# gardner-lab/syllable-detector-swift

Hardware: AMD Instinct MI355X
Metric: audio frames/sec (256-pt STFT + 2-layer MLP), whole job (higher is better)
Workload: dtype f32 (I/O and accumulate; products as f16 hi/lo split x3 on MFMA)

## Files before the change

syllable_detector_swift_amd/csrc/kernels_fused_s.hip:

```cpp

#include "fused_common.hpp"

namespace sd {

namespace {

using namespace fused_dev;

constexpr int kTile = kFusedSTileFrames;

typedef __attribute__((address_space(3))) void lds_void;

__device__ __forceinline__ float rem_lo(float a, unsigned h)
{
    float r;
    asm("v_fma_mix_f32 %0, %1, 1.0, -%2 op_sel_hi:[0,0,1]" : "=v"(r) : "v"(a), "v"(h));
    return r;
}
__device__ __forceinline__ float rem_hi(float a, unsigned h)
{
    float r;
    asm("v_fma_mix_f32 %0, %1, 1.0, -%2 op_sel:[0,0,1] op_sel_hi:[0,0,1]" : "=v"(r) : "v"(a), "v"(h));
    return r;
}
__device__ __forceinline__ unsigned cvt_pk(float a, float b)
{
    unsigned r;
    asm("v_cvt_pk_f16_f32 %0, %1, %2" : "=v"(r) : "v"(a), "v"(b));
    return r;
}
__device__ __forceinline__ floatx4 s16x4(const int16_t *p)
{
    const uint2 v = *reinterpret_cast<const uint2 *>(p);
    constexpr float k = 1.0f / 32768.0f;
    return floatx4{(float)(int16_t)(v.x & 0xffffu) * k, (float)((int)v.x >> 16) * k, (float)(int16_t)(v.y & 0xffffu) * k,
                   (float)((int)v.y >> 16) * k};
}
__device__ __forceinline__ float s16x1(const int16_t *p) { return (float)p[0] * (1.0f / 32768.0f); }

__device__ __forceinline__ void split2(float a, float b, unsigned &hi, unsigned &lo)
{
    hi = cvt_pk(a, b);
    lo = cvt_pk(rem_lo(a, hi), rem_hi(b, hi));
}

template <int K2, bool GEN, int HQ, int NW, int PADP = 0, bool F2 = false, int NT = 1, bool SPECT = false, bool MN = false, bool S16 = false>
__global__ void __launch_bounds__(64 * NW, 1)
fused_s_kernel(const FusedDesc d, const float *__restrict__ samples, int64_t stride, int64_t s_eff, int64_t E,
               float *__restrict__ outputs, uint8_t *__restrict__ flags, const FusedNet *__restrict__ nets, const int *__restrict__ net_of,
               const int *__restrict__ row_of)
{
    static_assert(!(MN && SPECT), "the spectrogram instantiation runs no network");
    static_assert(!S16 || (K2 == 4 && F2 && PADP == 0 && NT == 1 && HQ == 1 && NW == 8 && !SPECT), "16-bit PCM: the twice-folded form on the plain ring");
    extern __shared__ __attribute__((aligned(16))) unsigned char smem[];
    const int tid = threadIdx.x;
    const int lane = tid & 63;
    const int wave = __builtin_amdgcn_readfirstlane(tid >> 6);
    const int n = lane & 15, g = lane >> 4;
    constexpr int kWaves = NW;
    const int c = blockIdx.y;
    const int T = d.T, H = d.H, hop = d.hop;
    constexpr int W = 64 * K2;
    const int n_out = GEN ? d.n_out : 1;
    const int64_t e_b = ((int64_t)blockIdx.x * kWaves + wave) * d.s_seg_evals;
    if (e_b >= E) return;
    const int64_t e_e = (e_b + d.s_seg_evals < E) ? e_b + d.s_seg_evals : E;
    const int seg_len = (int)(e_e - e_b);
    const int tiles = (seg_len + (T - 1) + kTile - 1) / kTile;
    const unsigned e_b32 = (unsigned)e_b;
    const FusedNet *nt = MN ? nets + __builtin_amdgcn_readfirstlane(net_of[c]) : nullptr;
#define SD_NET(f) (MN ? nt->f : d.f)

    const int fr = d.s_perm ? (n < 4 ? 2 * n : (n >= 12 ? 2 * (n - 8) : 2 * (n - 4) + 1)) : n;

    unsigned char *wbase = smem + (size_t)wave * d.s_lds_wave;
    const int RC = PADP == 1 ? d.s_cs8_rc : d.s_ring_chunks, R = RC * (S16 ? 512 : 256);
    constexpr bool CS8 = PADP == 1;
    static_assert(!CS8 || (F2 && HQ == 1 && NT == 1), "staggered chunks: the twice-folded form at hop 128");
    constexpr int kSub = PADP > 1 ? 256 / PADP : 1;
    constexpr int kChunkB = CS8 ? 1280 : 1024 + (PADP > 1 ? 16 * kSub : 0);
    auto sk = [](int i) { return PADP > 1 ? 4 * (i / (PADP > 1 ? PADP : 1)) : 0; };
    float *ring = reinterpret_cast<float *>(wbase);
    const int16_t *ring16 = reinterpret_cast<const int16_t *>(wbase);
    const int PS = d.s_pstride, TP = d.s_tp;
    float *rows = reinterpret_cast<float *>(wbase + (size_t)(RC + (CS8 ? 0 : 1)) * kChunkB);
    float *zquad = rows + (T - 1 + kTile) * PS;
    constexpr bool kTbl = HQ == 2 && NW == 8;
    float *gtab = zquad + 8 * HQ + 32 * g;
    {
        const int nz = ((T - 1 + kTile) * PS + 8 * HQ + 128) / 4;
        for (int i = lane; i < nz; i += 64) reinterpret_cast<floatx4 *>(rows)[i] = floatx4{0.f, 0.f, 0.f, 0.f};
    }

    constexpr int KB = F2 ? 1 : K2;
    half8 as_[KB][2][2], ad_[KB][2][2];
    if (!F2) {
#pragma unroll
        for (int ks = 0; ks < KB; ks++)
#pragma unroll
            for (int m = 0; m < 2; m++)
#pragma unroll
                for (int p = 0; p < 2; p++) {
                    as_[ks][m][p] = as_half8(reinterpret_cast<const uint32x4 *>(d.sfrag)[(((ks * 2 + 0) * 2 + m) * 2 + p) * 64 + lane]);
                    ad_[ks][m][p] = as_half8(reinterpret_cast<const uint32x4 *>(d.sfrag)[(((ks * 2 + 1) * 2 + m) * 2 + p) * 64 + lane]);
                }
    }
    half8 b2[F2 ? 2 : 1][F2 ? 4 * NT : 1][2];
    float w1c[F2 ? 16 : 1], w2c[F2 ? 16 : 1], ce[4 * NT], w192 = 0.0f;
#pragma unroll
    for (int i = 0; i < 4 * NT; i++) ce[i] = 0.0f;
    if (F2) {
#pragma unroll
        for (int ks = 0; ks < 2; ks++)
#pragma unroll
            for (int gm = 0; gm < 4; gm++)
#pragma unroll
                for (int tau = 0; tau < NT; tau++)
#pragma unroll
                    for (int p = 0; p < 2; p++)
                        b2[ks][gm + 4 * tau][p] = as_half8(reinterpret_cast<const uint32x4 *>(d.sfrag2)[(((ks * 4 + gm) * NT + tau) * 2 + p) * 64 + lane]);
#pragma unroll
        for (int i = 0; i < 16; i++) {
            w1c[i] = d.swin2[(g * 16 + i) * 2];
            w2c[i] = d.swin2[(g * 16 + i) * 2 + 1];
        }
#pragma unroll
        for (int i = 0; i < 4 * NT; i++) ce[i] = d.s2c[lane * 16 + i];
        w192 = d.s2c[lane * 16 + 8];
    }
    half8 aft[3][HQ][NT][2];
#pragma unroll
    for (int m = 0; m < 3; m++)
#pragma unroll
        for (int q = 0; q < HQ; q++)
#pragma unroll
            for (int tau = 0; tau < NT; tau++)
#pragma unroll
                for (int p = 0; p < 2; p++)
                    aft[m][q][tau][p] = as_half8(reinterpret_cast<const uint32x4 *>(F2 ? (HQ == 1 ? SD_NET(afrag_t2) : SD_NET(afrag_w2)) : (HQ == 1 ? SD_NET(afrag_t) : SD_NET(afrag_w)))[(((m * HQ + q) * NT + tau) * 2 + p) * 64 + lane]);
    float cre[8];
#pragma unroll
    for (int i = 0; i < 8; i++) cre[i] = F2 ? 0.0f : d.slone[lane * 8 + i];
    if (kTbl && n == 0) {
#pragma unroll
        for (int i = 0; i < 8; i++) gtab[i] = cre[i];
    }

    const int rc = MN ? bank_row(row_of, c) : c;
    const float *row = S16 ? reinterpret_cast<const float *>(reinterpret_cast<const int16_t *>(samples) + (int64_t)rc * stride)
                           : samples + (int64_t)rc * stride;
    const __amdgpu_buffer_rsrc_t in_rs = __builtin_amdgcn_make_buffer_rsrc(const_cast<float *>(row), 0, (int)(s_eff * (S16 ? 2 : 4)), 0x00020000);
    const __amdgpu_buffer_rsrc_t out_rs = __builtin_amdgcn_make_buffer_rsrc(
        outputs ? outputs + (int64_t)rc * E * n_out : nullptr, 0, outputs ? (int)(E * n_out * 4) : 0, 0x00020000);
    const __amdgpu_buffer_rsrc_t flg_rs = __builtin_amdgcn_make_buffer_rsrc(flags ? flags + (int64_t)rc * E : nullptr, 0, flags ? (int)E : 0, 0x00020000);
    const __amdgpu_buffer_rsrc_t spc_rs = __builtin_amdgcn_make_buffer_rsrc(
        SPECT ? d.spect_out + (int64_t)c * E * d.F : nullptr, 0, SPECT ? (int)(E * d.F * 4) : 0, 0x00020000);

    const unsigned org = (unsigned)((e_b * hop + d.gap) * (S16 ? 2 : 4));
    int cn = 0, slot = 0;
    auto issue_upto = [&](int last) {
        while (cn <= last) {
            const unsigned voff = org + (unsigned)cn * 1024u + (unsigned)lane * 16u;
            if (CS8) {
                const int pad = ((cn & 6) << 1) | (cn & 1);
                __builtin_amdgcn_raw_ptr_buffer_load_lds(in_rs, (lds_void *)(wbase + slot * kChunkB + 16 * pad), 16, voff, 0, 0, 2 );
            } else if (PADP == 0) {
                __builtin_amdgcn_raw_ptr_buffer_load_lds(in_rs, (lds_void *)(wbase + slot * 1024), 16, voff, 0, 0, 2 );
                if (slot == 0) __builtin_amdgcn_raw_ptr_buffer_load_lds(in_rs, (lds_void *)(wbase + RC * 1024), 16, voff, 0, 0, 2);
            } else {
#pragma unroll
                for (int k = 0; k < kSub; k++)
                    if (lane / (64 / kSub) == k) {
                        __builtin_amdgcn_raw_ptr_buffer_load_lds(in_rs, (lds_void *)(wbase + slot * kChunkB + 16 * k), 16, voff, 0, 0, 2);
                        if (slot == 0) __builtin_amdgcn_raw_ptr_buffer_load_lds(in_rs, (lds_void *)(wbase + RC * kChunkB + 16 * k), 16, voff, 0, 0, 2);
                    }
            }
            cn++;
            slot = slot + 1 == RC ? 0 : slot + 1;
        }
    };
    const int span = (kTile - 1) * hop + W;
    constexpr int kChunkLog = S16 ? 9 : 8;
    auto need = [&](int t) { return (kTile * hop * t + span - 1) >> kChunkLog; };
    auto allowed = [&](int t) { return RC - 1 + ((kTile * hop * t) >> kChunkLog); };

    unsigned fo = (unsigned)(hop * fr);
    unsigned sb1 = (unsigned)((fr >> 1) * kChunkB), sb2 = (unsigned)(((fr >> 1) + (fr & 1)) * kChunkB);
    const int jq1 = (fr >> 1) & 7, jq2 = ((fr >> 1) + (fr & 1)) & 7;
    const unsigned cb1 = (unsigned)(16 * (((jq1 & 6) << 1) | (jq1 & 1)) + ((fr & 1) ? 512 : 0));
    const unsigned cb2 = (unsigned)(16 * (((jq2 & 6) << 1) | (jq2 & 1)) + ((fr & 1) ? 0 : 512));
    float *prow = rows + (T - 1 + fr) * PS;
    const float *erow = rows + n * PS;
    const float *pv_p[3], *sv_p[3];
#pragma unroll
    for (int tt = 0; tt < 3; tt++) {
        const int t = g + 4 * tt;
        pv_p[tt] = t < T ? erow + t * PS + 4 * HQ * t : zquad;
        sv_p[tt] = t < T ? erow + t * PS + 4 * HQ * TP : zquad;
    }
    float *pt_p[3];
#pragma unroll
    for (int m = 0; m < 3; m++) pt_p[m] = 4 * m + g < TP ? prow + 4 * HQ * (4 * m + g) : zquad + 4 * HQ;

    const float c_b1 = GEN ? (g < n_out ? SD_NET(b1)[g] : 0.0f) : SD_NET(b1)[0];
    float lean_oa = 0.0f, lean_og = 1.0f, lean_ob = 0.0f;
    if (d.n_out_fns == 1) {
        const int o = (GEN && g < n_out) ? g : 0;
        lean_oa = SD_NET(out_params)[0]; lean_og = SD_NET(out_params)[1 + o]; lean_ob = SD_NET(out_params)[1 + n_out + o];
    }
    float b0g[HQ], w1g[HQ], w1o[4][HQ], rvg[HQ];
#pragma unroll
    for (int q = 0; q < HQ; q++) {
        const int u = 4 * q + g;
        rvg[q] = (GEN && u < H) ? SD_NET(rvec)[u] : 0.0f;
        b0g[q] = u < H ? SD_NET(bias0)[u] : 0.0f;
        w1g[q] = u < H ? SD_NET(w1)[u] : 0.0f;
#pragma unroll
        for (int o = 0; o < 4; o++) w1o[o][q] = (GEN && u < H && o < n_out) ? SD_NET(w1)[o * H + u] : 0.0f;
    }
    if (kTbl && n == 0) {
#pragma unroll
        for (int q = 0; q < HQ; q++) {
            gtab[8 + q] = b0g[q];
            gtab[8 + HQ + q] = w1g[q];
            gtab[8 + 6 * HQ + q] = rvg[q];
#pragma unroll
            for (int o = 0; o < 4; o++) gtab[8 + 2 * HQ + o * HQ + q] = w1o[o][q];
        }
    }
    const bool multi = GEN && n_out > 1;
    const double thr_g = SD_NET(thresholds)[(GEN && g < n_out) ? g : 0];
    if (kTbl && n == 0) {
        gtab[22] = c_b1; gtab[23] = lean_oa; gtab[24] = lean_og; gtab[25] = lean_ob;
        *reinterpret_cast<double *>(gtab + 26) = thr_g;
    }
    const bool counts = !GEN || n_out == 1 ? true : (g < n_out && (g == 0 || d.rule == 1));
    const int tf0 = GEN ? d.tf0 : 0, tf1 = GEN ? d.tf1 : 2, norm = GEN ? d.norm : 1;
    const int scaling = GEN ? d.scaling : 0;
    const float klog = scaling == 1 ? 0.6931471805599453f : 6.020599913279624f;
    bool binv[8 * NT];
#pragma unroll
    for (int i = 0; i < 8 * NT; i++) {
        const int tau = i >> 3, ii = i & 7;
        binv[i] = (F2 ? 32 * tau + (ii < 4 ? 8 * g + d.s2_pe + 2 * ii : 8 * g + d.s2_po + 2 * (ii - 4)) : (ii < 4 ? 4 * g + ii : 16 + 4 * g + (ii - 4))) < d.F;
    }
    const float kmag = pow2f(-13 - d.col_shift);
    const bool guard_on = d.fix.counters != nullptr;
    const float guard_k = norm == 1 ? SD_NET(guard_r) : (norm == 0 ? SD_NET(guard_rel_r) : SD_NET(guard_range_r));
    const float mn_wu = MN ? nt->w_unscale : 0.0f, mn_loud = MN ? nt->guard_loud : 0.0f;
    const int mn_se_abs = MN ? nt->guard_se_abs_r : 0;
#undef SD_NET

    issue_upto(need(0) < allowed(0) ? need(0) : allowed(0));
    int se_ref = 0;

#ifdef SYLDET_S_STAMPS
    unsigned long long st_vm = 0, st_lg = 0;
    const unsigned long long st_begin = __builtin_amdgcn_s_memtime();
#define SD_STAMP(var, stmt) { asm volatile("s_waitcnt lgkmcnt(0)" ::: "memory"); const unsigned long long t0_ = __builtin_amdgcn_s_memtime(); stmt; \
                              const unsigned long long t1_ = __builtin_amdgcn_s_memtime(); var += t1_ - t0_; }
#else
#define SD_STAMP(var, stmt) { stmt; }
#endif
#ifndef SYLDET_S_NO_PREWAIT
    __builtin_amdgcn_s_waitcnt(0x0F70);
#endif
#if defined(SYLDET_S_SETPRIO_SECOND)
    if (wave >= kWaves / 2) __builtin_amdgcn_s_setprio(1);
#elif defined(SYLDET_S_SETPRIO_FIRST)
    if (wave < kWaves / 2) __builtin_amdgcn_s_setprio(1);
#endif
    for (int t = 0; t < tiles; t++) {
        SD_STAMP(st_vm, if (t == 0) asm volatile("s_waitcnt vmcnt(0)" ::: "memory"); else if (SPECT) asm volatile("s_waitcnt vmcnt(5)" ::: "memory");
                        else asm volatile("s_waitcnt vmcnt(2)" ::: "memory"));
        const float *f1 = reinterpret_cast<const float *>(wbase + sb1 + cb1);
        const float *f2 = reinterpret_cast<const float *>(wbase + sb2 + cb2);
        const float *fp = CS8 ? f1 : ring + fo + sk((int)fo);

        floatx4 P1[2][2], P3[2][2], P2[2][2], P4[2][2];
        float P2w[2], P4w[2], x64 = 0.0f, x192 = 0.0f;
        if (F2) {
#pragma unroll
            for (int ks = 0; ks < 2; ks++) {
                if (CS8) {
                    const float *a1 = f1 + 32 * ks + 8 * g, *a2 = f2 + 32 * ks + 8 * g;
                    const float *b1 = f1 + 120 - 32 * ks - 8 * g, *b3 = f2 + 120 - 32 * ks - 8 * g;
                    P1[ks][0] = *reinterpret_cast<const floatx4 *>(a1);
                    P1[ks][1] = *reinterpret_cast<const floatx4 *>(a1 + 4);
                    P3[ks][0] = *reinterpret_cast<const floatx4 *>(a2);
                    P3[ks][1] = *reinterpret_cast<const floatx4 *>(a2 + 4);
                    P2[ks][0] = *reinterpret_cast<const floatx4 *>(b1);
                    P2[ks][1] = *reinterpret_cast<const floatx4 *>(b1 + 4);
                    P2w[ks] = (ks == 0) ? (g == 0 ? f2 : b1 + 8)[0] : b1[8];
                    P4[ks][0] = *reinterpret_cast<const floatx4 *>(b3);
                    P4[ks][1] = *reinterpret_cast<const floatx4 *>(b3 + 4);
                    P4w[ks] = b3[8];
                    continue;
                }
                if (S16) {
                    const int16_t *a = ring16 + fo + 32 * ks + 8 * g, *b = ring16 + fo + 120 - 32 * ks - 8 * g;
                    P1[ks][0] = s16x4(a);
                    P1[ks][1] = s16x4(a + 4);
                    P3[ks][0] = s16x4(a + 128);
                    P3[ks][1] = s16x4(a + 132);
                    P2[ks][0] = s16x4(b);
                    P2[ks][1] = s16x4(b + 4);
                    P2w[ks] = s16x1(b + 8);
                    P4[ks][0] = s16x4(b + 128);
                    P4[ks][1] = s16x4(b + 132);
                    P4w[ks] = s16x1(b + 136);
                    continue;
                }
                const float *a = fp + 32 * ks + 8 * g, *b = fp + 120 - 32 * ks - 8 * g;
                P1[ks][0] = *reinterpret_cast<const floatx4 *>(a);
                P1[ks][1] = *reinterpret_cast<const floatx4 *>(a + 4);
                P3[ks][0] = *reinterpret_cast<const floatx4 *>(a + 128 + sk(128));
                P3[ks][1] = *reinterpret_cast<const floatx4 *>(a + 132 + sk(128));
                P2[ks][0] = *reinterpret_cast<const floatx4 *>(b + sk(64));
                P2[ks][1] = *reinterpret_cast<const floatx4 *>(b + 4 + sk(64));
                P2w[ks] = (PADP && ks == 0) ? b[8 + (g == 0 ? sk(128) : sk(64))] : b[8 + sk(64)];
                P4[ks][0] = *reinterpret_cast<const floatx4 *>(b + 128 + sk(192));
                P4[ks][1] = *reinterpret_cast<const floatx4 *>(b + 132 + sk(192));
                P4w[ks] = b[136 + sk(192)];
            }
            x64 = S16 ? s16x1(ring16 + fo + 64) : (CS8 ? f1[64] : fp[64 + sk(64)]);
            x192 = S16 ? s16x1(ring16 + fo + 192) : (CS8 ? f2[64] : fp[192 + sk(192)]);
            SD_STAMP(st_lg, asm volatile("s_waitcnt lgkmcnt(0)" ::: "memory"));
            if (t + 1 < tiles) issue_upto(need(t + 1));
        }
        float amax;
#ifdef SYLDET_S_NOMAX
        amax = 1.0f;
#else
        {
            float m0 = 0.0f, m1 = 0.0f;
            if (F2) {
#pragma unroll
                for (int ks = 0; ks < 2; ks++)
#pragma unroll
                    for (int h = 0; h < 2; h++) {
                        m0 = absmax3(m0, P1[ks][h][0], P1[ks][h][1]);
                        m1 = absmax3(m1, P1[ks][h][2], P1[ks][h][3]);
                        m0 = absmax3(m0, P3[ks][h][0], P3[ks][h][1]);
                        m1 = absmax3(m1, P3[ks][h][2], P3[ks][h][3]);
                        m0 = absmax3(m0, P2[ks][h][0], P2[ks][h][1]);
                        m1 = absmax3(m1, P2[ks][h][2], P2[ks][h][3]);
                        m0 = absmax3(m0, P4[ks][h][0], P4[ks][h][1]);
                        m1 = absmax3(m1, P4[ks][h][2], P4[ks][h][3]);
                    }
                m0 = absmax3(m0, P2w[0], P2w[1]);
                m1 = absmax3(m1, g == 0 ? 0.0f : P4w[0], P4w[1]);
                m0 = absmax3(m0, x64, x192);
            } else {
                const floatx4 *q0 = reinterpret_cast<const floatx4 *>(fp + (W / 4) * g + sk((W / 4) * g));
#pragma unroll
                for (int q = 0; q < W / 16; q++) {
                    const floatx4 v = q0[q];
                    m0 = absmax3(m0, v[0], v[1]);
                    m1 = absmax3(m1, v[2], v[3]);
                }
            }
            amax = fmaxf(m0, m1);
            auto r = __builtin_amdgcn_permlane16_swap(__float_as_uint(amax), __float_as_uint(amax), false, false);
            amax = fmaxf(__uint_as_float(r[0]), __uint_as_float(r[1]));
            r = __builtin_amdgcn_permlane32_swap(__float_as_uint(amax), __float_as_uint(amax), false, false);
            amax = fmaxf(__uint_as_float(r[0]), __uint_as_float(r[1]));
        }
#endif
        const int ex = (int)((__float_as_uint(amax) >> 23) & 0xffu);
        int se = (F2 ? 139 : 140) - ex;
        const int fst = amax > 0.0f ? ((ex == 255 || se < -100) ? 2 : 0) : 1;
        se = amax > 0.0f ? (se < -100 ? -100 : (se > 113 ? 113 : se)) : 0;
        const float sx = pow2f(se);
        if (t == 0) {
            const float tm = wave_max_nonneg(amax);
            const int exr = (int)((__float_as_uint(tm) >> 23) & 0xffu);
            int r0 = (F2 ? 139 : 140) - exr;
            r0 = tm > 0.0f ? (r0 < -100 ? -100 : (r0 > 113 ? 113 : r0)) : 0;
            se_ref = __builtin_amdgcn_readfirstlane(r0);
        }

        if (!F2 && t + 1 < tiles) issue_upto(need(t + 1) < allowed(t) ? need(t + 1) : allowed(t));

        const float xl = S16 ? 0.0f : fp[0] * sx;
        floatx4 acc[4 * NT];
#pragma unroll
        for (int i = 0; i < 4 * NT; i++) acc[i] = floatx4{0.f, 0.f, 0.f, 0.f};
        float a64 = 0.0f;
        const float *xpb = fp + W / 2 + 8 * g, *xmb = fp + W / 2 - 8 * g;
        const float *xmz = xmb + ((PADP && g == 0) ? 4 : 0);
#ifndef SYLDET_S_NODFT
        if (F2) {
            a64 = w192 * fmaf(x192, sx, x64 * sx);
            const float b64 = w192 * fmaf(x192, sx, -(x64 * sx));
#pragma unroll
            for (int ks = 0; ks < 2; ks++) {
                const float xa[8] = {P3[ks][0][0], P3[ks][0][1], P3[ks][0][2], P3[ks][0][3], P3[ks][1][0], P3[ks][1][1], P3[ks][1][2], P3[ks][1][3]};
                const float xd[8] = {P1[ks][0][0], P1[ks][0][1], P1[ks][0][2], P1[ks][0][3], P1[ks][1][0], P1[ks][1][1], P1[ks][1][2], P1[ks][1][3]};
                const float xb[8] = {P2w[ks], P2[ks][1][3], P2[ks][1][2], P2[ks][1][1], P2[ks][1][0], P2[ks][0][3], P2[ks][0][2], P2[ks][0][1]};
                const float xc[8] = {P4w[ks], P4[ks][1][3], P4[ks][1][2], P4[ks][1][1], P4[ks][1][0], P4[ks][0][3], P4[ks][0][2], P4[ks][0][1]};
                float ap[8], am[8], bm[8], bp[8];
#pragma unroll
                for (int i = 0; i < 8; i++) {
                    const float t1 = xb[i] * sx, t2 = xd[i] * sx;
                    float s1 = fmaf(xa[i], sx, t1), d1 = fmaf(xa[i], sx, -t1);
                    float s2 = fmaf(xc[i], sx, t2), d2 = fmaf(xc[i], sx, -t2);
                    if (ks == 0 && i == 0) {
                        s1 = g == 0 ? xa[0] * sx : s1;
                        s2 = g == 0 ? t2 : s2;
                    }
                    const float w1 = w1c[ks * 8 + i], w2 = w2c[ks * 8 + i];
                    const float p = w2 * s2, q = w2 * d2;
                    ap[i] = fmaf(w1, s1, p);
                    am[i] = fmaf(w1, s1, -p);
                    bm[i] = fmaf(w1, d1, -q);
                    bp[i] = fmaf(w1, d1, q);
                }
                if (ks == 0) {
                    bm[0] = g == 0 ? 0.0f : bm[0];
                    bp[0] = g == 0 ? b64 : bp[0];
                }
                uint32x4 vh[4], vl[4];
#pragma unroll
                for (int j = 0; j < 4; j++) {
                    unsigned h, l;
                    split2(ap[2 * j], ap[2 * j + 1], h, l);
                    vh[0][j] = h; vl[0][j] = l;
                    split2(am[2 * j], am[2 * j + 1], h, l);
                    vh[1][j] = h; vl[1][j] = l;
                    split2(bm[2 * j], bm[2 * j + 1], h, l);
                    vh[2][j] = h; vl[2][j] = l;
                    split2(bp[2 * j], bp[2 * j + 1], h, l);
                    vh[3][j] = h; vl[3][j] = l;
                }
#pragma unroll
                for (int gm = 0; gm < 4 * NT; gm++) acc[gm] = mfma(b2[ks][gm][0], as_half8(vh[gm & 3]), acc[gm]);
#pragma unroll
                for (int gm = 0; gm < 4 * NT; gm++) acc[gm] = mfma(b2[ks][gm][0], as_half8(vl[gm & 3]), acc[gm]);
#pragma unroll
                for (int gm = 0; gm < 4 * NT; gm++) acc[gm] = mfma(b2[ks][gm][1], as_half8(vh[gm & 3]), acc[gm]);
            }
        } else {
#pragma unroll
        for (int ks = 0; ks < KB; ks++) {
            const int skp = sk(W / 2 + 32 * ks), skm = sk(W / 2 - 32 * ks - 32), skw = sk(W / 2 - 32 * ks);
            const floatx4 p0 = *reinterpret_cast<const floatx4 *>(xpb + 32 * ks + skp), p1 = *reinterpret_cast<const floatx4 *>(xpb + 32 * ks + 4 + skp);
            const floatx4 q1 = *reinterpret_cast<const floatx4 *>(xmb - 32 * ks - 8 + skm), q2 = *reinterpret_cast<const floatx4 *>(xmb - 32 * ks - 4 + skm);
            const float q0 = (skw != skm ? xmz : xmb)[-32 * ks + skm];
            const float xp[8] = {p0[0], p0[1], p0[2], p0[3], p1[0], p1[1], p1[2], p1[3]};
            const float xm[8] = {q0, q2[3], q2[2], q2[1], q2[0], q1[3], q1[2], q1[1]};
            float s[8], dd[8];
#pragma unroll
            for (int i = 0; i < 8; i++) {
                const float tm = xm[i] * sx;
                s[i] = fmaf(xp[i], sx, tm);
                dd[i] = fmaf(xp[i], sx, -tm);
            }
            if (ks == 0) dd[0] = g == 0 ? xl : dd[0];
            uint32x4 sh, sl, dh, dl;
#pragma unroll
            for (int j = 0; j < 4; j++) {
                unsigned h, l;
                split2(s[2 * j], s[2 * j + 1], h, l);
                sh[j] = h; sl[j] = l;
                split2(dd[2 * j], dd[2 * j + 1], h, l);
                dh[j] = h; dl[j] = l;
            }
            const half8 bsh = as_half8(sh), bsl = as_half8(sl), bdh = as_half8(dh), bdl = as_half8(dl);
#pragma unroll
            for (int m = 0; m < 2; m++) acc[m] = mfma(as_[ks][m][0], bsh, acc[m]);
#pragma unroll
            for (int m = 0; m < 2; m++) acc[2 + m] = mfma(ad_[ks][m][0], bdh, acc[2 + m]);
#pragma unroll
            for (int m = 0; m < 2; m++) acc[m] = mfma(as_[ks][m][0], bsl, acc[m]);
#pragma unroll
            for (int m = 0; m < 2; m++) acc[2 + m] = mfma(ad_[ks][m][0], bdl, acc[2 + m]);
#pragma unroll
            for (int m = 0; m < 2; m++) acc[m] = mfma(as_[ks][m][1], bsh, acc[m]);
#pragma unroll
            for (int m = 0; m < 2; m++) acc[2 + m] = mfma(ad_[ks][m][1], bdh, acc[2 + m]);
        }
        }
#else
        acc[0][0] = xpb[0]; acc[1][1] = xmb[0];
#endif
        if (!F2) {
            SD_STAMP(st_lg, asm volatile("s_waitcnt lgkmcnt(0)" ::: "memory"));
            if (t + 1 < tiles) issue_upto(need(t + 1));
        }

        float cval[8 * NT], mss = 0.0f;
        float cre_l[8];
        if (kTbl) {
            const float *tp = gtab;
            asm volatile("" : "+v"(tp));
            const floatx4 c0 = *reinterpret_cast<const floatx4 *>(tp), c1 = *reinterpret_cast<const floatx4 *>(tp + 4);
#pragma unroll
            for (int i = 0; i < 4; i++) { cre_l[i] = c0[i]; cre_l[4 + i] = c1[i]; }
        } else {
#pragma unroll
            for (int i = 0; i < 8; i++) cre_l[i] = cre[i];
        }
#pragma unroll
        for (int i = 0; i < 8 * NT; i++) {
            const int tau = i >> 3, ii = i & 7;
            const float re = F2 ? (ii < 4 ? fmaf(ce[4 * tau + ii], a64, acc[4 * tau][ii]) : acc[4 * tau + 1][ii & 3]) : fmaf(cre_l[ii], xl, acc[ii >> 2][ii & 3]);
            const float im = F2 ? (ii < 4 ? acc[4 * tau + 2][ii] : acc[4 * tau + 3][ii & 3]) : acc[2 + (ii >> 2)][ii & 3];
            cval[i] = __builtin_amdgcn_sqrtf(fmaf(re, re, im * im)) * kmag;
        }
        if constexpr (SPECT) {
            static_assert(NT == 1 && F2, "the spectrogram instantiation is the twice-folded one");
            const int er = kTile * t + fr;
            const bool vld = er < seg_len;
            const int ush = d.col_shift - se;
            const float up = pow2f(ush < -126 ? -126 : (ush > 126 ? 126 : ush));
            const unsigned rowo = (e_b32 + (unsigned)er) * (unsigned)d.F;
            const bool odd_first = d.s2_pe != 0;
            float v8[8];
#pragma unroll
            for (int i = 0; i < 4; i++) {
                const float me = cval[i] * up, mo = cval[4 + i] * up;
                const float a = odd_first ? mo : me, b = odd_first ? me : mo;
                v8[2 * i] = d.spect_power ? a * a : a;
                v8[2 * i + 1] = d.spect_power ? b * b : b;
            }
            const int fq = d.F >> 2, rem = d.F & 3;
#pragma unroll
            for (int q = 0; q < 2; q++) {
                const int Q = 2 * g + q;
                const uint32x4 w = {__float_as_uint(v8[4 * q]), __float_as_uint(v8[4 * q + 1]), __float_as_uint(v8[4 * q + 2]), __float_as_uint(v8[4 * q + 3])};
                __builtin_amdgcn_raw_buffer_store_b128(w, spc_rs, (vld && Q < fq) ? (rowo + 4u * (unsigned)Q) * 4u : 0xFFFFFFFFu, 0, 0);
            }
            {
                const bool mine = vld && (fq >> 1) == g;
#pragma unroll
                for (int j = 0; j < 3; j++) {
                    const float pv = (fq & 1) ? v8[4 + j] : v8[j];
                    __builtin_amdgcn_raw_buffer_store_b32(__float_as_uint(pv), spc_rs, (mine && j < rem) ? (rowo + 4u * (unsigned)fq + (unsigned)j) * 4u : 0xFFFFFFFFu, 0, 0);
                }
            }
            if (guard_on && __builtin_amdgcn_ballot_w64(vld && fst == 2) != 0ull) {
                const int lo = kTile * t, hi = lo + kTile < seg_len ? lo + kTile : seg_len;
                if (lane == 0 && hi > lo) {
                    const unsigned sl = atomicAdd(d.fix.counters, 1u);
                    if (sl < d.fix.capacity) d.fix.items[sl] = FixItem{c, e_b32 + (unsigned)lo, hi - lo, 1};
                    else d.fix.counters[3] = 1u;
                }
            }
            fo += (unsigned)(kTile * hop);
            fo = fo >= (unsigned)R ? fo - (unsigned)R : fo;
            if (CS8) {
                sb1 += 8u * kChunkB; sb1 = sb1 >= (unsigned)(RC * kChunkB) ? sb1 - (unsigned)(RC * kChunkB) : sb1;
                sb2 += 8u * kChunkB; sb2 = sb2 >= (unsigned)(RC * kChunkB) ? sb2 - (unsigned)(RC * kChunkB) : sb2;
            }
            continue;
        }
        if (GEN && scaling != 0) {
            const float off = (float)(d.col_shift - se) * klog;
#pragma unroll
            for (int i = 0; i < 8 * NT; i++) cval[i] = binv[i] ? fmaf(__builtin_amdgcn_logf(cval[i]), klog, off) : 0.0f;
        }
#pragma unroll
        for (int i = 0; i < 8 * NT; i++) mss = fmaf(cval[i], cval[i], mss);
        mss = xor32_sum(xor16_sum(mss));
        int dsc = (GEN && scaling != 0) ? 0 : se_ref - se;
        const bool far = dsc > 45 || dsc < -45 || fst == 2;
        dsc = dsc < -45 ? -45 : (dsc > 45 ? 45 : dsc);
        unsigned tb = ((__float_as_uint(mss) + 0x800000u) >> 1) & 0x7f800000u;
        tb = (unsigned)min(max((int)tb, 16 << 23), 80 << 23);
        const float fs_up = __uint_as_float((203u << 23) - tb);
        const float fs_ring = __uint_as_float(tb + ((unsigned)(dsc + 51) << 23));
        uint32x4 bh[NT], bl[NT];
#pragma unroll
        for (int j = 0; j < 4 * NT; j++) {
            unsigned h, l;
            split2(cval[2 * j] * fs_up, cval[2 * j + 1] * fs_up, h, l);
            bh[j >> 2][j & 3] = h; bl[j >> 2][j & 3] = l;
        }
        floatx4 pt[3][HQ];
#pragma unroll
        for (int m = 0; m < 3; m++)
#pragma unroll
            for (int q = 0; q < HQ; q++) {
                pt[m][q] = floatx4{0.f, 0.f, 0.f, 0.f};
#pragma unroll
                for (int tau = 0; tau < NT; tau++) {
                    pt[m][q] = mfma(aft[m][q][tau][0], as_half8(bh[tau]), pt[m][q]);
                    pt[m][q] = mfma(aft[m][q][tau][0], as_half8(bl[tau]), pt[m][q]);
                    pt[m][q] = mfma(aft[m][q][tau][1], as_half8(bh[tau]), pt[m][q]);
                }
            }
#pragma unroll
        for (int m = 0; m < 3; m++)
#pragma unroll
            for (int q = 0; q < HQ; q++) *reinterpret_cast<floatx4 *>(pt_p[m] + 4 * q) = pt[m][q] * fs_ring;
        {
            float st0 = mss * pow2f(2 * dsc), st1 = 0.0f;
            if (GEN && norm == 2) {
                float mn = INFINITY, mx = -INFINITY;
#pragma unroll
                for (int i = 0; i < 8 * NT; i++) {
                    mn = binv[i] ? fminf(mn, cval[i]) : mn;
                    mx = binv[i] ? fmaxf(mx, cval[i]) : mx;
                }
                auto r = __builtin_amdgcn_permlane16_swap(__float_as_uint(mn), __float_as_uint(mn), false, false);
                mn = fminf(__uint_as_float(r[0]), __uint_as_float(r[1]));
                r = __builtin_amdgcn_permlane32_swap(__float_as_uint(mn), __float_as_uint(mn), false, false);
                mn = fminf(__uint_as_float(r[0]), __uint_as_float(r[1]));
                r = __builtin_amdgcn_permlane16_swap(__float_as_uint(mx), __float_as_uint(mx), false, false);
                mx = fmaxf(__uint_as_float(r[0]), __uint_as_float(r[1]));
                r = __builtin_amdgcn_permlane32_swap(__float_as_uint(mx), __float_as_uint(mx), false, false);
                mx = fmaxf(__uint_as_float(r[0]), __uint_as_float(r[1]));
                st0 = mn * pow2f(dsc);
                st1 = mx * pow2f(dsc);
            } else if (GEN && norm == 3) {
                float sm = 0.0f;
#pragma unroll
                for (int i = 0; i < 8 * NT; i++) sm += binv[i] ? cval[i] : 0.0f;
                sm = xor32_sum(xor16_sum(sm));
                const float mean = sm / (float)d.F;
                float m2 = 0.0f;
#pragma unroll
                for (int i = 0; i < 8 * NT; i++) {
                    const float dl = cval[i] - mean;
                    m2 = binv[i] ? fmaf(dl, dl, m2) : m2;
                }
                m2 = xor32_sum(xor16_sum(m2));
                st0 = mean * pow2f(dsc);
                st1 = m2 * pow2f(2 * dsc);
            }
            if (GEN && norm == 0) st1 = st0;
            const float fw = far ? INFINITY : ((fst == 1 || (GEN && scaling != 0)) ? 0.0f : pow2f(2 * dsc));
            if (g == 0) *reinterpret_cast<floatx4 *>(prow + 4 * HQ * TP) = floatx4{st0, fw, st1, 0.0f};
        }

        floatx4 zp[HQ];
        float ssp, fwp, st1p = 0.0f;
        float sq0[3];
        const int nq = (T - 1) * PS / 4;
        floatx4 cy0 = {0.f, 0.f, 0.f, 0.f}, cy1 = cy0, cy2 = cy0;
        if (HQ == 1) {
            const floatx4 *src = reinterpret_cast<const floatx4 *>(rows + kTile * PS);
            cy0 = src[lane < nq ? lane : 0];
            cy1 = src[lane + 64 < nq ? lane + 64 : 0];
            if (nq > 128) cy2 = src[lane + 128 < nq ? lane + 128 : 0];
        }
        {
            floatx4 pv[3][HQ];
#pragma unroll
            for (int tt = 0; tt < 3; tt++)
#pragma unroll
                for (int q = 0; q < HQ; q++) pv[tt][q] = *reinterpret_cast<const floatx4 *>(pv_p[tt] + 4 * q);
            const floatx4 s0 = *reinterpret_cast<const floatx4 *>(sv_p[0]), s1 = *reinterpret_cast<const floatx4 *>(sv_p[1]),
                          s2 = *reinterpret_cast<const floatx4 *>(sv_p[2]);
            sq0[0] = s0[0]; sq0[1] = s1[0]; sq0[2] = s2[0];
#pragma unroll
            for (int q = 0; q < HQ; q++) zp[q] = pv[0][q] + pv[1][q] + pv[2][q];
            if (GEN && (norm == 0 || norm == 2)) {
                ssp = fminf(fminf(g < T ? s0[0] : INFINITY, g + 4 < T ? s1[0] : INFINITY), g + 8 < T ? s2[0] : INFINITY);
                st1p = norm == 0 ? s0[2] + s1[2] + s2[2]
                                 : fmaxf(fmaxf(g < T ? s0[2] : -INFINITY, g + 4 < T ? s1[2] : -INFINITY), g + 8 < T ? s2[2] : -INFINITY);
            } else {
                ssp = s0[0] + s1[0] + s2[0];
                st1p = s0[2] + s1[2] + s2[2];
            }
            fwp = fmaxf(fmaxf(s0[1], s1[1]), s2[1]);
        }
        float zt[HQ], ssw, fww, st1w = 0.0f;
        {
#pragma unroll
            for (int q = 0; q < HQ; q++) {
                auto r = __builtin_amdgcn_permlane16_swap(__float_as_uint(zp[q][0]), __float_as_uint(zp[q][1]), false, false);
                const float s01 = __uint_as_float(r[0]) + __uint_as_float(r[1]);
                r = __builtin_amdgcn_permlane16_swap(__float_as_uint(zp[q][2]), __float_as_uint(zp[q][3]), false, false);
                const float s23 = __uint_as_float(r[0]) + __uint_as_float(r[1]);
                r = __builtin_amdgcn_permlane32_swap(__float_as_uint(s01), __float_as_uint(s23), false, false);
                zt[q] = __uint_as_float(r[0]) + __uint_as_float(r[1]);
            }
            auto r = __builtin_amdgcn_permlane16_swap(__float_as_uint(ssp), __float_as_uint(ssp), false, false);
            if (GEN && (norm == 0 || norm == 2)) {
                const float m = fminf(__uint_as_float(r[0]), __uint_as_float(r[1]));
                r = __builtin_amdgcn_permlane32_swap(__float_as_uint(m), __float_as_uint(m), false, false);
                ssw = fminf(__uint_as_float(r[0]), __uint_as_float(r[1]));
            } else {
                ssw = xor32_sum(__uint_as_float(r[0]) + __uint_as_float(r[1]));
            }
            if (GEN && norm == 2) {
                r = __builtin_amdgcn_permlane16_swap(__float_as_uint(st1p), __float_as_uint(st1p), false, false);
                const float m = fmaxf(__uint_as_float(r[0]), __uint_as_float(r[1]));
                r = __builtin_amdgcn_permlane32_swap(__float_as_uint(m), __float_as_uint(m), false, false);
                st1w = fmaxf(__uint_as_float(r[0]), __uint_as_float(r[1]));
            } else if (GEN && norm == 0) {
                st1w = xor32_sum(xor16_sum(st1p));
            } else if (GEN && norm == 3) {
                const float mean = ssw / (float)T;
                float dv = 0.0f;
#pragma unroll
                for (int tt = 0; tt < 3; tt++) {
                    const float dl = sq0[tt] - mean;
                    dv = g + 4 * tt < T ? fmaf(dl, dl, dv) : dv;
                }
                st1w = xor32_sum(xor16_sum(st1p)) + (float)d.F * xor32_sum(xor16_sum(dv));
                ssw = mean;
            }
            r = __builtin_amdgcn_permlane16_swap(__float_as_uint(fwp), __float_as_uint(fwp), false, false);
            const float m = fmaxf(__uint_as_float(r[0]), __uint_as_float(r[1]));
            r = __builtin_amdgcn_permlane32_swap(__float_as_uint(m), __float_as_uint(m), false, false);
            fww = fmaxf(__uint_as_float(r[0]), __uint_as_float(r[1]));
        }
        float yv, gstat = ssw;
        bool hit;
        {
            const int ush = (GEN && scaling != 0) ? 0 : d.col_shift - se_ref;
            const float alpha0 = (MN ? mn_wu : d.w_unscale) * pow2f(ush < -120 ? -120 : (ush > 120 ? 120 : ush));
            float alpha = norm == 1 ? (MN ? mn_wu : d.w_unscale) * __builtin_amdgcn_rsqf(ssw) : alpha0, beta = 0.0f;
            if (GEN && norm == 2) {
                const float range = st1w - ssw;
                gstat = range;
                if (range == 0.0f) { alpha = 0.0f; beta = -1.0f; }
                else { alpha = (MN ? mn_wu : d.w_unscale) * 2.0f / range; beta = (0.0f - ssw - st1w) / range; }
            } else if (GEN && norm == 3) {
                const float sdv = sqrtf(st1w / (float)d.I);
                gstat = sdv;
                alpha = (MN ? mn_wu : d.w_unscale) / sdv;
                beta = -ssw / sdv;
            }
            float b0_l[HQ], w1_l[HQ], w1o_l[4][HQ], rv_l[HQ];
            if (kTbl) {
                const float *tp = gtab + 8;
                asm volatile("" : "+v"(tp));
#pragma unroll
                for (int q = 0; q < HQ; q++) {
                    b0_l[q] = tp[q];
                    w1_l[q] = tp[HQ + q];
                    rv_l[q] = norm >= 2 ? tp[6 * HQ + q] : 0.0f;
#pragma unroll
                    for (int o = 0; o < 4; o++) w1o_l[o][q] = multi ? tp[2 * HQ + o * HQ + q] : 0.0f;
                }
            } else {
#pragma unroll
                for (int q = 0; q < HQ; q++) {
                    b0_l[q] = b0g[q];
                    w1_l[q] = w1g[q];
                    rv_l[q] = rvg[q];
#pragma unroll
                    for (int o = 0; o < 4; o++) w1o_l[o][q] = w1o[o][q];
                }
            }
            float act[HQ];
#pragma unroll
            for (int q = 0; q < HQ; q++)
                act[q] = transfer_fn(tf0, (GEN && norm >= 2) ? fmaf(alpha, zt[q], fmaf(beta, rv_l[q], b0_l[q])) : fmaf(alpha, zt[q], b0_l[q]));
            float ysum;
            if (multi) {
                float yp[4];
#pragma unroll
                for (int o = 0; o < 4; o++) {
                    yp[o] = w1o_l[o][0] * act[0];
#pragma unroll
                    for (int q = 1; q < HQ; q++) yp[o] = fmaf(w1o_l[o][q], act[q], yp[o]);
                }
                auto r = __builtin_amdgcn_permlane16_swap(__float_as_uint(yp[0]), __float_as_uint(yp[1]), false, false);
                const float a01 = __uint_as_float(r[0]) + __uint_as_float(r[1]);
                r = __builtin_amdgcn_permlane16_swap(__float_as_uint(yp[2]), __float_as_uint(yp[3]), false, false);
                const float a23 = __uint_as_float(r[0]) + __uint_as_float(r[1]);
                r = __builtin_amdgcn_permlane32_swap(__float_as_uint(a01), __float_as_uint(a23), false, false);
                ysum = __uint_as_float(r[0]) + __uint_as_float(r[1]);
            } else {
                float yq = w1_l[0] * act[0];
#pragma unroll
                for (int q = 1; q < HQ; q++) yq = fmaf(w1_l[q], act[q], yq);
                ysum = xor32_sum(xor16_sum(yq));
            }
            float ob1 = c_b1, ooa = lean_oa, oog = lean_og, oob = lean_ob;
            double othr = thr_g;
            if (kTbl) {
                const float *tp = gtab + 22;
                asm volatile("" : "+v"(tp));
                const floatx4 ov = *reinterpret_cast<const floatx4 *>(tp - 2);
                ob1 = ov[2]; ooa = ov[3];
                oog = tp[2]; oob = tp[3];
                othr = *reinterpret_cast<const double *>(tp + 4);
            }
            float y = transfer_fn(tf1, ysum + ob1);
            y = (y - ooa) / oog + oob;
            yv = y;
            hit = counts && (double)y >= othr;
            if (multi) {
                unsigned hb = hit ? 1u : 0u;
                auto r = __builtin_amdgcn_permlane16_swap(hb, hb, false, false);
                hb = r[0] | r[1];
                r = __builtin_amdgcn_permlane32_swap(hb, hb, false, false);
                hit = (r[0] | r[1]) != 0u;
            }
        }
        const int er = kTile * t - (T - 1) + n;
        const bool vld = er >= 0 && er < seg_len;
        {
            const bool st = vld && g == 0, sto = vld && g < n_out;
            const unsigned off = e_b32 + (unsigned)er;
            __builtin_amdgcn_raw_buffer_store_b32(__float_as_uint(yv), out_rs, sto ? (off * (unsigned)n_out + (unsigned)g) * 4u : 0xFFFFFFFFu, 0, 0);
            __builtin_amdgcn_raw_buffer_store_b8((unsigned char)(hit ? 1 : 0), flg_rs, st ? off : 0xFFFFFFFFu, 0, 0);
        }
        if (guard_on) {
            bool bad = vld && !(fww == 0.0f) && !(gstat >= guard_k * ((GEN && norm >= 2) ? sqrtf(fww) : fww));
            if (GEN && norm == 0 && fww != INFINITY && fww != 0.0f) {
                const int lg = (int)((__float_as_uint(fww) >> 23) & 0xffu) - 127;
                if (se_ref - lg / 2 >= (MN ? mn_se_abs : d.guard_se_abs_r)) bad = false;
            }
            if (GEN && norm == 0 && scaling == 0 && vld) {
                const int ush2 = 2 * (d.col_shift - se_ref);
                const float u2 = st1w * pow2f(ush2 < -120 ? -120 : (ush2 > 120 ? 120 : ush2));
                if (u2 * (MN ? mn_loud : d.guard_loud) > 1.0f) bad = true;
            }
            if (__builtin_amdgcn_ballot_w64(bad) != 0ull) {
                const int er0 = kTile * t - (T - 1);
                const int lo = er0 < 0 ? 0 : er0, hi = er0 + kTile < seg_len ? er0 + kTile : seg_len;
                if (lane == 0 && hi > lo) {
                    const unsigned sl = atomicAdd(d.fix.counters, 1u);
                    if (sl < d.fix.capacity) d.fix.items[sl] = FixItem{c, e_b32 + (unsigned)lo, hi - lo, 0};
                    else d.fix.counters[3] = 1u;
                }
            }
        }
        {
            floatx4 *dst = reinterpret_cast<floatx4 *>(rows);
            if (HQ == 1) {
                if (lane < nq) dst[lane] = cy0;
                if (lane + 64 < nq) dst[lane + 64] = cy1;
                if (nq > 128 && lane + 128 < nq) dst[lane + 128] = cy2;
            } else {
                const floatx4 *src = reinterpret_cast<const floatx4 *>(rows + kTile * PS);
                for (int i = lane; i < nq; i += 64) dst[i] = src[i];
            }
        }
        fo += (unsigned)(kTile * hop);
        fo = fo >= (unsigned)R ? fo - (unsigned)R : fo;
        if (CS8) {
            sb1 += 8u * kChunkB; sb1 = sb1 >= (unsigned)(RC * kChunkB) ? sb1 - (unsigned)(RC * kChunkB) : sb1;
            sb2 += 8u * kChunkB; sb2 = sb2 >= (unsigned)(RC * kChunkB) ? sb2 - (unsigned)(RC * kChunkB) : sb2;
        }
    }
#ifdef SYLDET_S_STAMPS
    if (d.stamps && lane == 0) {
        atomicAdd(d.stamps + 0, __builtin_amdgcn_s_memtime() - st_begin);
        atomicAdd(d.stamps + 1, st_vm);
        atomicAdd(d.stamps + 2, st_lg);
        atomicAdd(d.stamps + 3, (unsigned long long)tiles);
        atomicAdd(d.stamps + 4, 1ull);
    }
#endif
#undef SD_STAMP
}

template <int K2, bool GEN, int HQ, int NW, int PADP = 0, bool F2 = false, int NT = 1, bool SPECT = false, bool MN = false, bool S16 = false>
hipError_t launch_one(const FusedDesc &d, const float *samples, int64_t stride, int C, int64_t s_eff, int64_t E,
                      float *outputs, uint8_t *flags, hipStream_t stream, const FusedMulti *mn = nullptr)
{
    if constexpr (!SPECT && !MN)
        if (mn) return launch_one<K2, GEN, HQ, NW, PADP, F2, NT, false, true, S16>(d, samples, stride, C, s_eff, E, outputs, flags, stream, mn);
    auto kern = fused_s_kernel<K2, GEN, HQ, NW, PADP, F2, NT, SPECT, MN, S16>;
    constexpr int kWaves = NW;
#ifdef SYLDET_S_ONEWAVE
    const int lds = kWaves == 4 ? 100 * 1024 : d.s_lds_wave * kWaves;
#else
    const int lds = d.s_lds_wave * kWaves;
#endif
    hipError_t st = hipFuncSetAttribute((const void *)kern, hipFuncAttributeMaxDynamicSharedMemorySize, lds);
    if (st != hipSuccess) return st;
    const int64_t segs = (E + d.s_seg_evals - 1) / d.s_seg_evals;
    dim3 grid((unsigned)((segs + kWaves - 1) / kWaves), (unsigned)C);
    const FusedNet *nets = MN ? mn->nets : nullptr;
    const int *net_of = MN ? mn->net_of : nullptr;
    const int *row_of = MN ? mn->row_of : nullptr;
    hipLaunchKernelGGL(kern, grid, dim3(64 * kWaves), (size_t)lds, stream, d, samples, stride, s_eff, E, outputs, flags, nets, net_of, row_of);
    return hipGetLastError();
}

}

bool fused_s_has_stamps()
{
#ifdef SYLDET_S_STAMPS
    return true;
#else
    return false;
#endif
}

bool fused_s_applicable(const FusedDesc &d)
{
    const bool cls = d.norm >= 0 && d.norm <= 3 && d.n_layers == 2 && d.n_out >= 1 && d.n_out <= 4 && d.H <= 16 && d.n_out_fns <= 1;
    if (d.F > 32 && !(d.s2_ok && d.s2_nt == 2 && !d.no_fold2)) return false;
    return d.s_ok && d.T <= 12 && cls;
}

hipError_t launch_fused_s(const FusedDesc &d, const float *samples, int64_t stride, int C, int64_t S, int64_t J,
                          int64_t E, float *outputs, uint8_t *flags, hipStream_t stream, const FusedMulti *mn, bool s16)
{
    (void)S;
    if (E <= 0 || C <= 0) return hipSuccess;
    if (!fused_s_applicable(d)) return hipErrorInvalidValue;
    const int64_t s_eff = (J - 1) * (int64_t)d.hop + d.gap + d.W;
    if (s_eff * 4 >= 0x7fffffffll) return hipErrorInvalidValue;
    const bool exact = d.norm == 1 && d.scaling == 0 && d.tf0 == 0  && d.tf1 == 2  && d.n_out == 1;
    if (s16) {
        if (!fused_s_native_s16(d) || (reinterpret_cast<uintptr_t>(samples) & 3) != 0 || (stride & 1) != 0 || (d.gap & 1) != 0)
            return hipErrorInvalidValue;
        if (exact) return launch_one<4, false, 1, 8, 0, true, 1, false, false, true>(d, samples, stride, C, s_eff, E, outputs, flags, stream, mn);
        return launch_one<4, true, 1, 8, 0, true, 1, false, false, true>(d, samples, stride, C, s_eff, E, outputs, flags, stream, mn);
    }
#define SD_S_GO(K2_)                                                                                                  \
    if (d.W == 64 * K2_) {                                                                                            \
// ... 78 lines not shown
```

Before: 8.881 billion.

## Streamline DMA ring issue, carry-row copy addressing, and max reductions in fused kernel

Replaces the per-chunk recomputed DMA addresses and slot logic with incrementally advanced LDS and global offsets. The wrap-around duplicate chunk is now issued once per ring cycle instead of being checked on every chunk. Need/allowed bounds are tracked with running accumulators clamped to a precomputed end, which removes the per-tile multiplies and the t+1<tiles branches. It also drops the t==0 full vmcnt wait, precomputes branch-free LDS addresses for the carry-row copy, and does the max reductions as unsigned integer max on non-negative floats. These changes aim to cut scalar and VALU overhead in the hot loop, at the cost of subtler invariants around ring wrap and wait counts.

```diff
diff --git a/syllable_detector_swift_amd/csrc/kernels_fused_s.hip b/syllable_detector_swift_amd/csrc/kernels_fused_s.hip
--- a/syllable_detector_swift_amd/csrc/kernels_fused_s.hip
+++ b/syllable_detector_swift_amd/csrc/kernels_fused_s.hip
@@ -10,6 +10,7 @@
 constexpr int kTile = kFusedSTileFrames;
 
 typedef __attribute__((address_space(3))) void lds_void;
+typedef __attribute__((address_space(3))) floatx4 lds_floatx4;
 
 __device__ __forceinline__ float rem_lo(float a, unsigned h)
 {
@@ -37,6 +38,9 @@
                    (float)((int)v.y >> 16) * k};
 }
 __device__ __forceinline__ float s16x1(const int16_t *p) { return (float)p[0] * (1.0f / 32768.0f); }
+
+__device__ __forceinline__ float amax3(float m, float x, float y) { return fmaxf(fmaxf(fabsf(x), fabsf(y)), m); }
+__device__ __forceinline__ float umaxf(float a, float b) { return __uint_as_float(max(__float_as_uint(a), __float_as_uint(b))); }
 
 __device__ __forceinline__ void split2(float a, float b, unsigned &hi, unsigned &lo)
 {
@@ -157,38 +161,42 @@
         SPECT ? d.spect_out + (int64_t)c * E * d.F : nullptr, 0, SPECT ? (int)(E * d.F * 4) : 0, 0x00020000);
 
     const unsigned org = (unsigned)((e_b * hop + d.gap) * (S16 ? 2 : 4));
-    int cn = 0, slot = 0;
+    int cn = 0, cz = 0;
+    unsigned soff = 0, voff = org + (unsigned)lane * 16u;
+    const unsigned ring_b = (unsigned)RC * kChunkB;
+    auto dma = [&](unsigned lo, unsigned vo) {
+        if (PADP <= 1) {
+            __builtin_amdgcn_raw_ptr_buffer_load_lds(in_rs, (lds_void *)(wbase + lo), 16, vo, 0, 0, 2 );
+        } else {
+#pragma unroll
+            for (int k = 0; k < kSub; k++)
+                if (lane / (64 / kSub) == k)
+                    __builtin_amdgcn_raw_ptr_buffer_load_lds(in_rs, (lds_void *)(wbase + lo + 16 * k), 16, vo, 0, 0, 2 );
+        }
+    };
     auto issue_upto = [&](int last) {
+        if (!CS8 && cz <= last) {
+            dma(ring_b, voff + ((unsigned)(cz - cn) << 10));
+            cz += RC;
+        }
         while (cn <= last) {
-            const unsigned voff = org + (unsigned)cn * 1024u + (unsigned)lane * 16u;
-            if (CS8) {
-                const int pad = ((cn & 6) << 1) | (cn & 1);
-                __builtin_amdgcn_raw_ptr_buffer_load_lds(in_rs, (lds_void *)(wbase + slot * kChunkB + 16 * pad), 16, voff, 0, 0, 2 );
-            } else if (PADP == 0) {
-                __builtin_amdgcn_raw_ptr_buffer_load_lds(in_rs, (lds_void *)(wbase + slot * 1024), 16, voff, 0, 0, 2 );
-                if (slot == 0) __builtin_amdgcn_raw_ptr_buffer_load_lds(in_rs, (lds_void *)(wbase + RC * 1024), 16, voff, 0, 0, 2);
-            } else {
-#pragma unroll
-                for (int k = 0; k < kSub; k++)
-                    if (lane / (64 / kSub) == k) {
-                        __builtin_amdgcn_raw_ptr_buffer_load_lds(in_rs, (lds_void *)(wbase + slot * kChunkB + 16 * k), 16, voff, 0, 0, 2);
-                        if (slot == 0) __builtin_amdgcn_raw_ptr_buffer_load_lds(in_rs, (lds_void *)(wbase + RC * kChunkB + 16 * k), 16, voff, 0, 0, 2);
-                    }
-            }
+            dma(CS8 ? soff + (unsigned)(((cn & 7) + (cn & 6)) << 4) : soff, voff);
+            voff += 1024u;
             cn++;
-            slot = slot + 1 == RC ? 0 : slot + 1;
+            soff += (unsigned)kChunkB;
+            soff = soff == ring_b ? 0u : soff;
         }
     };
     const int span = (kTile - 1) * hop + W;
     constexpr int kChunkLog = S16 ? 9 : 8;
-    auto need = [&](int t) { return (kTile * hop * t + span - 1) >> kChunkLog; };
-    auto allowed = [&](int t) { return RC - 1 + ((kTile * hop * t) >> kChunkLog); };
+    const int tile_smp = kTile * hop;
+    int nacc = span - 1, aacc = 0;
+    const int need_end = (tile_smp * (tiles - 1) + span - 1) >> kChunkLog;
 
     unsigned fo = (unsigned)(hop * fr);
-    unsigned sb1 = (unsigned)((fr >> 1) * kChunkB), sb2 = (unsigned)(((fr >> 1) + (fr & 1)) * kChunkB);
     const int jq1 = (fr >> 1) & 7, jq2 = ((fr >> 1) + (fr & 1)) & 7;
-    const unsigned cb1 = (unsigned)(16 * (((jq1 & 6) << 1) | (jq1 & 1)) + ((fr & 1) ? 512 : 0));
-    const unsigned cb2 = (unsigned)(16 * (((jq2 & 6) << 1) | (jq2 & 1)) + ((fr & 1) ? 0 : 512));
+    unsigned sb1 = (unsigned)((fr >> 1) * kChunkB) + (unsigned)(16 * (((jq1 & 6) << 1) | (jq1 & 1)) + ((fr & 1) ? 512 : 0));
+    unsigned sb2 = (unsigned)(((fr >> 1) + (fr & 1)) * kChunkB) + (unsigned)(16 * (((jq2 & 6) << 1) | (jq2 & 1)) + ((fr & 1) ? 0 : 512));
     float *prow = rows + (T - 1 + fr) * PS;
     const float *erow = rows + n * PS;
     const float *pv_p[3], *sv_p[3];
@@ -201,6 +209,15 @@
     float *pt_p[3];
 #pragma unroll
     for (int m = 0; m < 3; m++) pt_p[m] = 4 * m + g < TP ? prow + 4 * HQ * (4 * m + g) : zquad + 4 * HQ;
+
+    const int nq = (T - 1) * PS / 4;
+    unsigned cya[3];
+#pragma unroll
+    for (int k = 0; k < 3; k++) {
+        const int i = lane + 64 * k;
+        cya[k] = i < nq ? lds_addr(rows) + 16u * (unsigned)i : (k ? cya[k - 1] : lds_addr(rows) + 16u * (unsigned)(nq + (lane & 31)));
+    }
+    const unsigned cy_src = (unsigned)(kTile * PS * 4);
 
     const float c_b1 = GEN ? (g < n_out ? SD_NET(b1)[g] : 0.0f) : SD_NET(b1)[0];
     float lean_oa = 0.0f, lean_og = 1.0f, lean_ob = 0.0f;
@@ -251,7 +268,7 @@
     const int mn_se_abs = MN ? nt->guard_se_abs_r : 0;
 #undef SD_NET
 
-    issue_upto(need(0) < allowed(0) ? need(0) : allowed(0));
+    issue_upto(min(min(nacc >> kChunkLog, need_end), RC - 1));
     int se_ref = 0;
 
 #ifdef SYLDET_S_STAMPS
@@ -271,10 +288,14 @@
     if (wave < kWaves / 2) __builtin_amdgcn_s_setprio(1);
 #endif
     for (int t = 0; t < tiles; t++) {
+#ifdef SYLDET_S_NO_PREWAIT
         SD_STAMP(st_vm, if (t == 0) asm volatile("s_waitcnt vmcnt(0)" ::: "memory"); else if (SPECT) asm volatile("s_waitcnt vmcnt(5)" ::: "memory");
                         else asm volatile("s_waitcnt vmcnt(2)" ::: "memory"));
-        const float *f1 = reinterpret_cast<const float *>(wbase + sb1 + cb1);
-        const float *f2 = reinterpret_cast<const float *>(wbase + sb2 + cb2);
+#else
+        SD_STAMP(st_vm, if (SPECT) asm volatile("s_waitcnt vmcnt(5)" ::: "memory"); else asm volatile("s_waitcnt vmcnt(2)" ::: "memory"));
+#endif
+        const float *f1 = reinterpret_cast<const float *>(wbase + sb1);
+        const float *f2 = reinterpret_cast<const float *>(wbase + sb2);
         const float *fp = CS8 ? f1 : ring + fo + sk((int)fo);
 
         floatx4 P1[2][2], P3[2][2], P2[2][2], P4[2][2];
@@ -326,7 +347,8 @@
             x64 = S16 ? s16x1(ring16 + fo + 64) : (CS8 ? f1[64] : fp[64 + sk(64)]);
             x192 = S16 ? s16x1(ring16 + fo + 192) : (CS8 ? f2[64] : fp[192 + sk(192)]);
             SD_STAMP(st_lg, asm volatile("s_waitcnt lgkmcnt(0)" ::: "memory"));
-            if (t + 1 < tiles) issue_upto(need(t + 1));
+            nacc += tile_smp;
+            issue_upto(min(nacc >> kChunkLog, need_end));
         }
         float amax;
 #ifdef SYLDET_S_NOMAX
@@ -339,32 +361,32 @@
                 for (int ks = 0; ks < 2; ks++)
 #pragma unroll
                     for (int h = 0; h < 2; h++) {
-                        m0 = absmax3(m0, P1[ks][h][0], P1[ks][h][1]);
-                        m1 = absmax3(m1, P1[ks][h][2], P1[ks][h][3]);
-                        m0 = absmax3(m0, P3[ks][h][0], P3[ks][h][1]);
-                        m1 = absmax3(m1, P3[ks][h][2], P3[ks][h][3]);
-                        m0 = absmax3(m0, P2[ks][h][0], P2[ks][h][1]);
-                        m1 = absmax3(m1, P2[ks][h][2], P2[ks][h][3]);
-                        m0 = absmax3(m0, P4[ks][h][0], P4[ks][h][1]);
-                        m1 = absmax3(m1, P4[ks][h][2], P4[ks][h][3]);
+                        m0 = amax3(m0, P1[ks][h][0], P1[ks][h][1]);
+                        m1 = amax3(m1, P1[ks][h][2], P1[ks][h][3]);
+                        m0 = amax3(m0, P3[ks][h][0], P3[ks][h][1]);
+                        m1 = amax3(m1, P3[ks][h][2], P3[ks][h][3]);
+                        m0 = amax3(m0, P2[ks][h][0], P2[ks][h][1]);
+                        m1 = amax3(m1, P2[ks][h][2], P2[ks][h][3]);
+                        m0 = amax3(m0, P4[ks][h][0], P4[ks][h][1]);
+                        m1 = amax3(m1, P4[ks][h][2], P4[ks][h][3]);
                     }
-                m0 = absmax3(m0, P2w[0], P2w[1]);
-                m1 = absmax3(m1, g == 0 ? 0.0f : P4w[0], P4w[1]);
-                m0 = absmax3(m0, x64, x192);
+                m0 = amax3(m0, P2w[0], P2w[1]);
+                m1 = amax3(m1, g == 0 ? 0.0f : P4w[0], P4w[1]);
+                m0 = amax3(m0, x64, x192);
             } else {
                 const floatx4 *q0 = reinterpret_cast<const floatx4 *>(fp + (W / 4) * g + sk((W / 4) * g));
 #pragma unroll
                 for (int q = 0; q < W / 16; q++) {
                     const floatx4 v = q0[q];
-                    m0 = absmax3(m0, v[0], v[1]);
-                    m1 = absmax3(m1, v[2], v[3]);
+                    m0 = amax3(m0, v[0], v[1]);
+                    m1 = amax3(m1, v[2], v[3]);
                 }
             }
             amax = fmaxf(m0, m1);
             auto r = __builtin_amdgcn_permlane16_swap(__float_as_uint(amax), __float_as_uint(amax), false, false);
-            amax = fmaxf(__uint_as_float(r[0]), __uint_as_float(r[1]));
-            r = __builtin_amdgcn_permlane32_swap(__float_as_uint(amax), __float_as_uint(amax), false, false);
-            amax = fmaxf(__uint_as_float(r[0]), __uint_as_float(r[1]));
+            unsigned um = max(r[0], r[1]);
+            r = __builtin_amdgcn_permlane32_swap(um, um, false, false);
+            amax = __uint_as_float(max(r[0], r[1]));
         }
 #endif
         const int ex = (int)((__float_as_uint(amax) >> 23) & 0xffu);
@@ -380,7 +402,11 @@
             se_ref = __builtin_amdgcn_readfirstlane(r0);
         }
 
-        if (!F2 && t + 1 < tiles) issue_upto(need(t + 1) < allowed(t) ? need(t + 1) : allowed(t));
+        if (!F2) {
+            nacc += tile_smp;
+            issue_upto(min(min(nacc >> kChunkLog, need_end), RC - 1 + (aacc >> kChunkLog)));
+            aacc += tile_smp;
+        }
 
         const float xl = S16 ? 0.0f : fp[0] * sx;
         floatx4 acc[4 * NT];
@@ -486,7 +512,7 @@
 #endif
         if (!F2) {
             SD_STAMP(st_lg, asm volatile("s_waitcnt lgkmcnt(0)" ::: "memory"));
-            if (t + 1 < tiles) issue_upto(need(t + 1));
+            issue_upto(min(nacc >> kChunkLog, need_end));
         }
 
         float cval[8 * NT], mss = 0.0f;
@@ -631,19 +657,24 @@
             }
             if (GEN && norm == 0) st1 = st0;
             const float fw = far ? INFINITY : ((fst == 1 || (GEN && scaling != 0)) ? 0.0f : pow2f(2 * dsc));
-            if (g == 0) *reinterpret_cast<floatx4 *>(prow + 4 * HQ * TP) = floatx4{st0, fw, st1, 0.0f};
+#ifdef SYLDET_S_STAT_DUMP
+            *reinterpret_cast<floatx4 *>(g == 0 ? prow + 4 * HQ * TP : zquad + 4 * HQ) = floatx4{st0, fw, st1, 0.0f};
+#else
+            *reinterpret_cast<floatx4 *>(prow + 4 * HQ * TP) = floatx4{st0, fw, st1, 0.0f};
+#endif
         }
 
         floatx4 zp[HQ];
         float ssp, fwp, st1p = 0.0f;
         float sq0[3];
-        const int nq = (T - 1) * PS / 4;
-        floatx4 cy0 = {0.f, 0.f, 0.f, 0.f}, cy1 = cy0, cy2 = cy0;
+        floatx4 cy[3] = {{0.f, 0.f, 0.f, 0.f}, {0.f, 0.f, 0.f, 0.f}, {0.f, 0.f, 0.f, 0.f}};
         if (HQ == 1) {
-            const floatx4 *src = reinterpret_cast<const floatx4 *>(rows + kTile * PS);
-            cy0 = src[lane < nq ? lane : 0];
-            cy1 = src[lane + 64 < nq ? lane + 64 : 0];
-            if (nq > 128) cy2 = src[lane + 128 < nq ? lane + 128 : 0];
+#pragma unroll
+            for (int k = 0; k < 3; k++) {
+                unsigned a = cya[k];
+                asm volatile("" : "+v"(a));
+                cy[k] = *reinterpret_cast<const lds_floatx4 *>(a + cy_src);
+            }
         }
         {
             floatx4 pv[3][HQ];
@@ -664,7 +695,7 @@
                 ssp = s0[0] + s1[0] + s2[0];
                 st1p = s0[2] + s1[2] + s2[2];
             }
-            fwp = fmaxf(fmaxf(s0[1], s1[1]), s2[1]);
+            fwp = umaxf(umaxf(s0[1], s1[1]), s2[1]);
         }
         float zt[HQ], ssw, fww, st1w = 0.0f;
         {
@@ -704,9 +735,9 @@
                 ssw = mean;
             }
             r = __builtin_amdgcn_permlane16_swap(__float_as_uint(fwp), __float_as_uint(fwp), false, false);
-            const float m = fmaxf(__uint_as_float(r[0]), __uint_as_float(r[1]));
-            r = __builtin_amdgcn_permlane32_swap(__float_as_uint(m), __float_as_uint(m), false, false);
-            fww = fmaxf(__uint_as_float(r[0]), __uint_as_float(r[1]));
+            const unsigned m = max(r[0], r[1]);
+            r = __builtin_amdgcn_permlane32_swap(m, m, false, false);
+            fww = __uint_as_float(max(r[0], r[1]));
         }
         float yv, gstat = ssw;
         bool hit;
@@ -826,9 +857,8 @@
         {
             floatx4 *dst = reinterpret_cast<floatx4 *>(rows);
             if (HQ == 1) {
-                if (lane < nq) dst[lane] = cy0;
-                if (lane + 64 < nq) dst[lane + 64] = cy1;
-                if (nq > 128 && lane + 128 < nq) dst[lane + 128] = cy2;
+#pragma unroll
+                for (int k = 0; k < 3; k++) *reinterpret_cast<lds_floatx4 *>(cya[k]) = cy[k];
             } else {
                 const floatx4 *src = reinterpret_cast<const floatx4 *>(rows + kTile * PS);
                 for (int i = lane; i < nq; i += 64) dst[i] = src[i];
```

After: 8.910 billion, median of 6. About the same (+0.3%).
